# achao2013/deep3dmap

Measured on AMD Instinct MI355X. Metric: rendered Mpix/s fwd+bwd, 100k-tri mesh @512x512, higher is better.
Workload: dtype f32

## Files before the change

deep3dmap_amd/csrc/d3m_face_major.h:

```cpp
#pragma once
#include "d3m_backward.h"
#include "d3m_forward.h"

namespace d3m {

#ifndef D3M_FM_MAX_BBOX_AREA
#define D3M_FM_MAX_BBOX_AREA 4096
#endif
constexpr int FM_MAX_BBOX_AREA = D3M_FM_MAX_BBOX_AREA;
constexpr int FM_LANES = 8;
constexpr int FM_FACES_PER_BLOCK = 256 / FM_LANES;

template <int N>
struct BoxCursorN {
    int x, y, x0, x1, bw;
    __device__ __forceinline__ BoxCursorN(int x0_, int x1_, int y0_, int start) : x0(x0_), x1(x1_), bw(x1_ - x0_ + 1) {
        y = y0_ + start / bw;
        x = x0_ + start % bw;
    }
    __device__ __forceinline__ void advance() {
        x += N;
        while (x > x1) { x -= bw; y++; }
    }
};
typedef BoxCursorN<FM_LANES> BoxCursor;

__device__ __forceinline__ float quad_sum(float v) {
    static_assert(FM_LANES == 8, "quad_sum is written for 8 lanes per face");
    v += dpp_f32<0xB1>(v);
    v += dpp_f32<0x4E>(v);
    v += dpp_f32<0x141>(v);
    return v;
}
constexpr int FLAG_HIDDEN = 0, FLAG_VISIBLE = 1, FLAG_LARGE = 2;

__global__ void __launch_bounds__(256) k_mark_visible(const int32_t* __restrict__ face_index_map, int* __restrict__ flags,
                                                     int B, int F, int S) {
    const long i = (long)blockIdx.x * 256 + threadIdx.x;
    if (i >= (long)B * S * S) return;
    const int fi = face_index_map[i];
    if (fi >= 0) flags[(size_t)(i / ((long)S * S)) * F + fi] = FLAG_VISIBLE;
}

template <class FS, int LANES>
__device__ __forceinline__ void backward_depth_face(FS fs, const float* __restrict__ depth_map,
                                                    const int32_t* __restrict__ face_index_map,
                                                    const float* __restrict__ weight_map,
                                                    const float* __restrict__ grad_depth_map, float* __restrict__ grad_faces,
                                                    int* __restrict__ flags, int S, long gi, int sub, int F,
                                                    const VertexTarget& vt, int* __restrict__ n_large, int flip_rows,
                                                    int max_area) {
    const int bn = (int)(gi / F), fn = (int)(gi % F);
    float face[9], finv[9];
    fs.load(bn, fn, face);
    int x0, x1, y0, y1;
    if (!pixel_bbox(face, S, x0, x1, y0, y1)) return;
    const int area = (x1 - x0 + 1) * (y1 - y0 + 1);
    if (area > max_area) {
        flags[gi] = FLAG_LARGE;
        if (n_large && sub == 0) atomicAdd(n_large, 1);
        return;
    }
    face_inverse(face, S, finv);
    float tmp[3] = {0, 0, 0};
#pragma unroll
    for (int k = 0; k < 3; k++) {
#pragma unroll
        for (int l = 0; l < 3; l++) tmp[k] += -finv[3 * l + k] / face[3 * l + 2];
    }
    float acc[9] = {0, 0, 0, 0, 0, 0, 0, 0, 0};
    const size_t base = (size_t)bn * S * S;
    BoxCursorN<LANES> c(x0, x1, y0, sub);
    for (int i = sub; i < area; i += LANES, c.advance()) {
        const size_t p = base + (size_t)c.y * S + c.x;
        const bool own = face_index_map[p] == fn;
        const float ld = depth_map[p], lg = grad_depth_map[flip_rows ? base + (size_t)(S - 1 - c.y) * S + c.x : p];
        const float lw[3] = {weight_map[3 * p], weight_map[3 * p + 1], weight_map[3 * p + 2]};
        if (!__builtin_amdgcn_ballot_w64(own)) continue;
        const float depth = own ? ld : 1.0f, g = own ? lg : 0.0f;
        const float depth2 = depth * depth;
#pragma unroll
        for (int k = 0; k < 3; k++) {
            const float wk = own ? lw[k] : 0.0f, z_k = face[3 * k + 2];
            acc[3 * k + 0] += -g * tmp[0] * wk * depth2 * (float)S / 2.0f;
            acc[3 * k + 1] += -g * tmp[1] * wk * depth2 * (float)S / 2.0f;
            acc[3 * k + 2] += g * wk * depth2 / (z_k * z_k);
        }
    }
#pragma unroll
    for (int k = 0; k < 9; k++) acc[k] = LANES == 64 ? wave_sum(acc[k]) : quad_sum(acc[k]);
    if (sub == 0) {
        if (vt.gv) {
#pragma unroll
            for (int v = 0; v < 3; v++) {
                float* g = vt.vertex(bn, fn, v);
#pragma unroll
                for (int k = 0; k < 3; k++) atomicAdd(&g[k], acc[3 * v + k]);
            }
        } else {
            float* gf = grad_faces + (size_t)gi * 9;
#pragma unroll
            for (int k = 0; k < 9; k++) gf[k] += acc[k];
        }
    }
}

template <class FS, int LANES = FM_LANES>
__global__ void __launch_bounds__(256) k_backward_depth_faces(FS fs, const float* __restrict__ depth_map,
                                                             const int32_t* __restrict__ face_index_map,
                                                             const float* __restrict__ weight_map,
                                                             const float* __restrict__ grad_depth_map,
                                                             float* __restrict__ grad_faces, int* __restrict__ flags, int B,
                                                             int S, const int* __restrict__ list,
                                                             const int* __restrict__ n_list, VertexTarget vt,
                                                             int* __restrict__ n_large, int flip_rows, int max_area) {
    static_assert(LANES == FM_LANES || LANES == 64, "eight lanes per face, or a wave");
    const int sub = threadIdx.x % LANES;
    const int F = fs.num_faces();
    const long n_units = list ? (long)*n_list : (long)B * F;
    for (long u = (long)blockIdx.x * (256 / LANES) + threadIdx.x / LANES; u < n_units; u += (long)gridDim.x * (256 / LANES)) {
        const long gi = list ? (long)list[u] : u;
        if (!list && flags[gi] == FLAG_HIDDEN) continue;
        backward_depth_face<FS, LANES>(fs, depth_map, face_index_map, weight_map, grad_depth_map, grad_faces, flags, S, gi, sub, F, vt,
                            n_large, flip_rows, max_area);
    }
}

template <class FS>
__global__ void __launch_bounds__(256) k_backward_textures_faces(FS fs, const int32_t* __restrict__ face_index_map,
                                                                const float* __restrict__ sampling_weight_map,
                                                                const int32_t* __restrict__ sampling_index_map,
                                                                const float* __restrict__ grad_rgb_map,
                                                                float* __restrict__ grad_textures, int* __restrict__ flags,
                                                                int B, int S) {
    __shared__ float s_acc[24][256];
    const long gi = (long)blockIdx.x * FM_FACES_PER_BLOCK + threadIdx.x / FM_LANES;
    const int sub = threadIdx.x % FM_LANES;
    const int F = fs.num_faces();
    if (gi >= (long)B * F || flags[gi] == FLAG_HIDDEN) return;
    const int bn = (int)(gi / F), fn = (int)(gi % F);
    float face[9];
    fs.load(bn, fn, face);
    int x0, x1, y0, y1;
    if (!pixel_bbox(face, S, x0, x1, y0, y1)) return;
    const int area = (x1 - x0 + 1) * (y1 - y0 + 1);
    if (area > FM_MAX_BBOX_AREA) { flags[gi] = FLAG_LARGE; return; }
    const int l = threadIdx.x;
#pragma unroll
    for (int t = 0; t < 24; t++) s_acc[t][l] = 0;
    const size_t base = (size_t)bn * S * S;
    BoxCursor c(x0, x1, y0, sub);
    for (int i = sub; i < area; i += FM_LANES, c.advance()) {
        const size_t p = base + (size_t)c.y * S + c.x;
        if (face_index_map[p] != fn) continue;
        const float g0 = grad_rgb_map[3 * p + 0], g1 = grad_rgb_map[3 * p + 1], g2 = grad_rgb_map[3 * p + 2];
#pragma unroll
        for (int pn = 0; pn < 8; pn++) {
            const float w = sampling_weight_map[p * 8 + pn];
            const int isc = sampling_index_map[p * 8 + pn] & 7;
            s_acc[isc * 3 + 0][l] += w * g0;
            s_acc[isc * 3 + 1][l] += w * g1;
            s_acc[isc * 3 + 2][l] += w * g2;
        }
    }
    __builtin_amdgcn_fence(__ATOMIC_RELEASE, "wavefront");
    __builtin_amdgcn_wave_barrier();
    __builtin_amdgcn_fence(__ATOMIC_ACQUIRE, "wavefront");
    if (sub == 0) {
        float* gt = grad_textures + (size_t)gi * 24;
#pragma unroll
        for (int t = 0; t < 24; t++) {
            float v = s_acc[t][l];
#pragma unroll
            for (int j = 1; j < FM_LANES; j++) v += s_acc[t][l + j];
            gt[t] += v;
        }
    }
}

}
```

deep3dmap_amd/csrc/d3m_lit.h:

```cpp
#pragma once
#include "d3m_aux.h"
#include "d3m_tail.h"
#include "d3m_face_major.h"

namespace d3m {

struct LitTextures {
    const float* textures;
    const float* light;
    int F, Fp, ts, tex_batch, light_batch, fill_back;
    const float* im;
    int im_H, im_W;
};

__device__ __forceinline__ long lit_texel(const LitTextures& t, int B, int b, int fp, int isc, int* light_row) {
    const int ts3 = t.ts * t.ts * t.ts;
    long vf = (long)b * t.Fp + fp + isc / ts3;
    isc %= ts3;
    if (vf >= (long)B * t.Fp) return -1;
    const int bb = (int)(vf / t.Fp), ff = (int)(vf % t.Fp);
    *light_row = (t.light_batch > 1 ? bb : 0) * t.Fp + ff;
    int fo = ff, idx = isc;
    if (ff >= t.F) {
        fo = ff - t.F;
// ... 616 lines not shown
        }
    }
    const float4 t = block_sum4_256(make_float4(t_rgb, t_d, t_m, t_sse), s_part);
    if (threadIdx.x == 0)
        reinterpret_cast<float4*>(fit.partials)[((size_t)blockIdx.z * gridDim.y + blockIdx.y) * gridDim.x + blockIdx.x] = t;
}

template <int TILE>
__global__ void __launch_bounds__(256) k_fit_loss_records(const float* __restrict__ rgb_im, const float* __restrict__ depth_im,
                                                         const float* __restrict__ alpha_im,
                                                         const int32_t* __restrict__ face_index_map, int B, int S,
                                                         FitTargets fit, FitRecords rec) {
    constexpr int ROWS = 256 / TILE;
    __shared__ float4 s_part[4];
    __shared__ int s_col_lo_inv[TILE], s_col_hi1[TILE];
    if (threadIdx.x < TILE) { s_col_lo_inv[threadIdx.x] = 0; s_col_hi1[threadIdx.x] = 0; }
    __syncthreads();
    const int b = blockIdx.z, x0 = blockIdx.x * TILE, y0 = blockIdx.y * TILE;
    const int tx = threadIdx.x % TILE, ty = threadIdx.x / TILE;
    const float inv_pixels = 1.0f / (float)((long)S * S), inv_3den = 1.0f / (3.0f * *rec.mask_sum);
    float t_rgb = 0, t_d = 0, t_m = 0, t_sse = 0;
    auto sgn = [](float x) { return x > 0 ? 1.0f : (x < 0 ? -1.0f : 0.0f); };
    for (int r = ty; r < TILE; r += ROWS) {
        const int yi = y0 + r, xi = x0 + tx;
        bool nz = false;
        if (yi < S && xi < S) {
            const int yo = S - 1 - yi;
            const size_t p = ((size_t)b * S + yi) * S + xi, o = ((size_t)b * S + yo) * S + xi;
            float tg[6], v[3];
#pragma unroll
            for (int k = 0; k < 3; k++) {
                tg[k] = fit.rgb_t[(((size_t)b * 3 + k) * S + yo) * S + xi];
                v[k] = rgb_im[(((size_t)b * 3 + k) * S + yo) * S + xi];
            }
            tg[3] = fit.depth_t[o]; tg[4] = fit.alpha_t[o]; tg[5] = fit.mask[o];
            const int fi = face_index_map[p];
            const float depth = depth_im[o], alpha = alpha_im[o];
            const float m = tg[5], d = alpha - tg[4];
#pragma unroll
            for (int k = 0; k < 3; k++) t_rgb += fabsf(v[k] - tg[k]) * m;
            t_d += fabsf(depth - tg[3]) * m;
            t_m += m;
            t_sse += d * d;
            float4 g;
            g.x = (2.0f * d) * inv_pixels;
            g.y = (sgn(v[0] - tg[0]) * m) * inv_3den;
            g.z = (sgn(v[1] - tg[1]) * m) * inv_3den;
            g.w = (sgn(v[2] - tg[2]) * m) * inv_3den;
            float dot = alpha * g.x;
            dot += v[0] * g.y;
            dot += v[1] * g.z;
            dot += v[2] * g.w;
            rec.grad[p] = g;
            rec.dot[p] = make_float2(dot, __int_as_float(fi));
            rec.g_depth[p] = sgn(depth - tg[3]) * m;
            nz = g.x != 0 || g.y != 0 || g.z != 0 || g.w != 0 || dot != 0;
        }
        const unsigned half = tile_row_mask<TILE>(__ballot(nz));
        if (half != 0 && tx == 0) {
            const size_t line = ((size_t)b * 2 + 1) * S + (y0 + r);
            atomicMax(&rec.nz_lo_inv[line], S - (x0 + (__ffs((int)half) - 1)));
            atomicMax(&rec.nz_hi1[line], x0 + (32 - __clz((int)half)));
        }
        if (nz) {
            atomicMax(&s_col_lo_inv[tx], S - (y0 + r));
            atomicMax(&s_col_hi1[tx], y0 + r + 1);
        }
    }
    __syncthreads();
    if (threadIdx.x < TILE && s_col_hi1[threadIdx.x] != 0 && x0 + (int)threadIdx.x < S) {
        const size_t line = ((size_t)b * 2 + 0) * S + (x0 + threadIdx.x);
        atomicMax(&rec.nz_lo_inv[line], s_col_lo_inv[threadIdx.x]);
        atomicMax(&rec.nz_hi1[line], s_col_hi1[threadIdx.x]);
    }
    const float4 t = block_sum4_256(make_float4(t_rgb, t_d, t_m, t_sse), s_part);
    if (threadIdx.x == 0)
        reinterpret_cast<float4*>(fit.partials)[((size_t)blockIdx.z * gridDim.y + blockIdx.y) * gridDim.x + blockIdx.x] = t;
}

#ifndef D3M_LIT_LANES
#define D3M_LIT_LANES 8
#endif
constexpr int LIT_LANES = D3M_LIT_LANES;
constexpr int LIT_FACES_PER_BLOCK = 256 / LIT_LANES;
__device__ __forceinline__ float lit_sum(float v) {
    v += dpp_f32<0xB1>(v);
    v += dpp_f32<0x4E>(v);
    if (LIT_LANES == 8) v += dpp_f32<0x141>(v);
    return v;
}

struct LitFaceArgs {
    const float* faces;
    LitTextures lt;
    const int32_t* face_index_map;
    const float *weight_map, *depth_map;
    RgbGrad grad_rgb;
    float* gtex_view;
    float* grad_light;
    const float* grad_depth_map;
    float* grad_faces;
    VertexTarget vt;
    int* flags;
    unsigned* view_mask;
    const int* list;
    const int* n_list;
    int B, S;
    float eps;
    GradScale gs;
    int* n_large;
    int max_area = FM_MAX_BBOX_AREA;
};

template <int LANES>
__device__ __forceinline__ float lit_lanes_sum(float v) { return LANES == 64 ? wave_sum(v) : lit_sum(v); }
template <int LANES>
__device__ __forceinline__ void lit_face_backward(const LitFaceArgs& a, long gi, int sub) {
    const float* __restrict__ faces = a.faces;
    const LitTextures& lt = a.lt;
    const int32_t* __restrict__ face_index_map = a.face_index_map;
    const float* __restrict__ weight_map = a.weight_map;
    const float* __restrict__ depth_map = a.depth_map;
    const RgbGrad grad_rgb = a.grad_rgb;
    float* __restrict__ gtex_view = a.gtex_view;
    float* __restrict__ grad_light = a.grad_light;
    const float* __restrict__ grad_depth_map = a.grad_depth_map;
    float* __restrict__ grad_faces = a.grad_faces;
    const VertexTarget& vt = a.vt;
    int* __restrict__ flags = a.flags;
    const int S = a.S;
    const float eps = a.eps;
    const int Fp = lt.Fp;
    float s_rgb, s_alpha, s_depth;
    a.gs.get(s_rgb, s_alpha, s_depth);
    if (!a.list && flags[gi] == FLAG_HIDDEN) return;
    const int bn = (int)(gi / Fp), fn = (int)(gi % Fp);
    const float* face = faces + (size_t)gi * 9;
    float fc[9];
#pragma unroll
    for (int k = 0; k < 9; k++) fc[k] = face[k];
    int x0, x1, y0, y1;
    if (!pixel_bbox(fc, S, x0, x1, y0, y1)) return;
    const int area = (x1 - x0 + 1) * (y1 - y0 + 1);
    const int fo = fn >= lt.F ? fn - lt.F : fn;
    float* gt = gtex_view + ((size_t)bn * lt.F + fo) * 24;
    if (sub == 0 && a.view_mask) atomicOr(&a.view_mask[(size_t)fo * ((a.B + 31) >> 5) + (bn >> 5)], 1u << (bn & 31));
    if (area > a.max_area) {
        flags[gi] = FLAG_LARGE;
        if (sub == 0) atomicAdd(a.n_large, 1);
        for (int t = sub; t < 24; t += LANES) gt[t] = 0.0f;
        return;
    }
    float acc[24];
#pragma unroll
    for (int t = 0; t < 24; t++) acc[t] = 0.0f;
    const size_t base = (size_t)bn * S * S;
    float dacc[9] = {0, 0, 0, 0, 0, 0, 0, 0, 0}, dtmp[3] = {0, 0, 0};
    const float rz[3] = {__builtin_amdgcn_rcpf(fc[2]), __builtin_amdgcn_rcpf(fc[5]), __builtin_amdgcn_rcpf(fc[8])};
    if (grad_depth_map) {
        float px[3], py[3];
#pragma unroll
        for (int n = 0; n < 3; n++) { px[n] = to_pixel(fc[3 * n], S); py[n] = to_pixel(fc[3 * n + 1], S); }
        const float rden = __builtin_amdgcn_rcpf(px[2] * (py[0] - py[1]) + px[0] * (py[1] - py[2]) + px[1] * (py[2] - py[0]));
        const float ix[3] = {(py[1] - py[2]) * rden, (py[2] - py[0]) * rden, (py[0] - py[1]) * rden};
        const float iy[3] = {(px[2] - px[1]) * rden, (px[0] - px[2]) * rden, (px[1] - px[0]) * rden};
#pragma unroll
        for (int l2 = 0; l2 < 3; l2++) {
            dtmp[0] += -ix[l2] * rz[l2];
            dtmp[1] += -iy[l2] * rz[l2];
        }
    }
    const int lrow = (lt.light_batch > 1 ? bn : 0) * Fp + fn;
    const float li[3] = {lt.light[3 * (size_t)lrow], lt.light[3 * (size_t)lrow + 1], lt.light[3 * (size_t)lrow + 2]};
    constexpr int TPL = LANES >= 8 ? 1 : 8 / LANES;
    const float* tex_face = lt.textures + ((size_t)(lt.tex_batch > 1 ? bn : 0) * lt.F + fo) * 24;
    int to[TPL];
    float tx[TPL][3];
#pragma unroll
    for (int j = 0; j < TPL; j++) {
        const int t = (sub + j * LANES) & 7;
        to[j] = fn >= lt.F ? ((t & 1) << 2) | (t & 2) | ((t >> 2) & 1) : t;
#pragma unroll
        for (int c3 = 0; c3 < 3; c3++) tx[j][c3] = tex_face[to[j] * 3 + c3];
    }
    BoxCursorN<LANES> c(x0, x1, y0, sub);
    for (int i = sub; i < area; i += LANES, c.advance()) {
        const size_t p = base + (size_t)c.y * S + c.x;
        const bool own = face_index_map[p] == fn;
        const float lw0 = weight_map[3 * p], lw1 = weight_map[3 * p + 1], lw2 = weight_map[3 * p + 2];
        const float lg0 = grad_rgb.get(p, 0) * s_rgb, lg1 = grad_rgb.get(p, 1) * s_rgb, lg2 = grad_rgb.get(p, 2) * s_rgb;
        const float ld = depth_map[p], lgd = grad_depth_map ? grad_depth_map[p] * s_depth : 0.0f;
        if (!__builtin_amdgcn_ballot_w64(own)) continue;
        const float third = 1.0f / 3.0f;
        const float weight[3] = {own ? lw0 : third, own ? lw1 : third, own ? lw2 : third};
        const float g0 = own ? lg0 : 0.0f, g1 = own ? lg1 : 0.0f, g2 = own ? lg2 : 0.0f;
        const float depth = own ? ld : 1.0f;
        if (grad_depth_map) {
            const float g = own ? lgd : 0.0f, depth2 = depth * depth;
#pragma unroll
            for (int k = 0; k < 3; k++) {
                const float z_k = fc[3 * k + 2];
                dacc[3 * k + 0] += -g * dtmp[0] * weight[k] * depth2 * (float)S / 2.0f;
                dacc[3 * k + 1] += -g * dtmp[1] * weight[k] * depth2 * (float)S / 2.0f;
                dacc[3 * k + 2] += g * weight[k] * depth2 * (rz[k] * rz[k]);
            }
        }
        int fl[3] = {0, 0, 0};
        float fr[3];
#pragma unroll
        for (int k = 0; k < 3; k++) fr[k] = fminf(fmaxf(weight[k] * (depth * rz[k]), 0.0f), 1.0f - eps);
#pragma unroll
        for (int pn = 0; pn < 8; pn++) {
            float w;
            int isc_dyn;
            sample_corner(pn, 2, fl, fr, w, isc_dyn);
            const int isc = ((pn & 1) << 2) | (pn & 2) | ((pn >> 2) & 1);
            acc[isc * 3 + 0] += w * g0;
            acc[isc * 3 + 1] += w * g1;
            acc[isc * 3 + 2] += w * g2;
        }
    }
#pragma unroll
    for (int t = 0; t < 24; t++) acc[t] = lit_lanes_sum<LANES>(acc[t]);
    if (grad_depth_map) {
#pragma unroll
        for (int k = 0; k < 9; k++) dacc[k] = lit_lanes_sum<LANES>(dacc[k]);
        if (sub == 0) {
            if (vt.gv) {
#pragma unroll
                for (int n = 0; n < 3; n++) {
                    float* g = vt.vertex(bn, fn, n);
#pragma unroll
                    for (int k = 0; k < 3; k++) atomicAdd(&g[k], dacc[3 * n + k]);
                }
            } else {
                float* gf = grad_faces + (size_t)gi * 9;
#pragma unroll
                for (int k = 0; k < 9; k++) gf[k] += dacc[k];
            }
        }
    }
    float gl[3] = {0, 0, 0};
#pragma unroll
    for (int j = 0; j < TPL; j++) {
        float mine[3] = {0, 0, 0};
#pragma unroll
        for (int t = 0; t < 8; t++) {
            if (sub + j * LANES == t) { mine[0] = acc[3 * t]; mine[1] = acc[3 * t + 1]; mine[2] = acc[3 * t + 2]; }
        }
        if (sub + j * LANES < 8) {
#pragma unroll
            for (int c3 = 0; c3 < 3; c3++) {
                gt[to[j] * 3 + c3] = mine[c3] * li[c3];
                gl[c3] += mine[c3] * tx[j][c3];
            }
        }
    }
#pragma unroll
    for (int c3 = 0; c3 < 3; c3++) gl[c3] = lit_lanes_sum<LANES>(gl[c3]);
    if (grad_light && sub == 0) {
        atomicAdd(&grad_light[3 * (size_t)lrow + 0], gl[0]);
        atomicAdd(&grad_light[3 * (size_t)lrow + 1], gl[1]);
        atomicAdd(&grad_light[3 * (size_t)lrow + 2], gl[2]);
    }
}

template <int LANES = LIT_LANES>
__global__ void __launch_bounds__(256) k_backward_textures_lit_faces(LitFaceArgs a) {
    static_assert(LANES == LIT_LANES || LANES == 64, "LIT_LANES lanes per face, or a wave");
    constexpr int PER_BLOCK = 256 / LANES;
    const int sub = threadIdx.x % LANES, slot = threadIdx.x / LANES;
    if (a.list) {
        const int n = *a.n_list;
        const XcdOrder xo((n + PER_BLOCK - 1) / PER_BLOCK);
        for (int i = blockIdx.x; xo.more(i); i += gridDim.x) {
            const long base = (long)xo.unit(i) * PER_BLOCK;
            if (base + slot < n) lit_face_backward<LANES>(a, a.list[base + slot], sub);
        }
    } else {
        const long gi = (long)blockIdx.x * PER_BLOCK + slot;
        if (gi < (long)a.B * a.lt.Fp) lit_face_backward<LANES>(a, gi, sub);
    }
}

constexpr int LIT_ANY_MAX_TEXELS = 64;
template <int LANES>
__device__ __forceinline__ void lit_face_backward_any(const LitFaceArgs& a, long gi, int sub, float* __restrict__ acc_lds) {
    const LitTextures& lt = a.lt;
    const int S = a.S, Fp = lt.Fp, ts = lt.ts, ts3 = ts * ts * ts;
    float s_rgb, s_alpha, s_depth;
    a.gs.get(s_rgb, s_alpha, s_depth);
    const int bn = (int)(gi / Fp), fn = (int)(gi % Fp);
    float fc[9];
#pragma unroll
    for (int k = 0; k < 9; k++) fc[k] = a.faces[(size_t)gi * 9 + k];
    int x0, x1, y0, y1;
    if (!pixel_bbox(fc, S, x0, x1, y0, y1)) return;
    const int area = (x1 - x0 + 1) * (y1 - y0 + 1);
    const bool back = fn >= lt.F;
    const int fo = back ? fn - lt.F : fn;
    float* gt = a.gtex_view + ((size_t)bn * lt.F + fo) * ts3 * 3;
    if (sub == 0 && a.view_mask) atomicOr(&a.view_mask[(size_t)fo * ((a.B + 31) >> 5) + (bn >> 5)], 1u << (bn & 31));
    if (area > a.max_area) {
        a.flags[gi] = FLAG_LARGE;
        if (sub == 0) atomicAdd(a.n_large, 1);
        for (int t = sub; t < ts3 * 3; t += LANES) gt[t] = 0.0f;
        return;
    }
    for (int t = sub; t < ts3 * 3; t += LANES) acc_lds[t] = 0.0f;
    float dacc[9] = {0, 0, 0, 0, 0, 0, 0, 0, 0}, dtmp[3] = {0, 0, 0};
    if (a.grad_depth_map) {
        float finv[9];
        face_inverse(fc, S, finv);
#pragma unroll
        for (int k = 0; k < 3; k++) {
#pragma unroll
            for (int l = 0; l < 3; l++) dtmp[k] += -finv[3 * l + k] / fc[3 * l + 2];
        }
    }
    const int lrow = (lt.light_batch > 1 ? bn : 0) * Fp + fn;
    const float li[3] = {lt.light[3 * (size_t)lrow], lt.light[3 * (size_t)lrow + 1], lt.light[3 * (size_t)lrow + 2]};
    const float* tex_face = lt.textures + ((size_t)(lt.tex_batch > 1 ? bn : 0) * lt.F + fo) * ts3 * 3;
    __builtin_amdgcn_fence(__ATOMIC_RELEASE, "wavefront");
    __builtin_amdgcn_wave_barrier();
    const size_t base = (size_t)bn * S * S;
    BoxCursorN<LANES> c(x0, x1, y0, sub);
    for (int i = sub; i < area; i += LANES, c.advance()) {
        const size_t p = base + (size_t)c.y * S + c.x;
        const bool own = a.face_index_map[p] == fn;
        const float lw[3] = {a.weight_map[3 * p], a.weight_map[3 * p + 1], a.weight_map[3 * p + 2]};
        const float lg[3] = {a.grad_rgb.get(p, 0) * s_rgb, a.grad_rgb.get(p, 1) * s_rgb, a.grad_rgb.get(p, 2) * s_rgb};
        const float ld = a.depth_map[p], lgd = a.grad_depth_map ? a.grad_depth_map[p] * s_depth : 0.0f;
        if (!own) continue;
        if (a.grad_depth_map) {
            const float depth2 = ld * ld;
#pragma unroll
            for (int k = 0; k < 3; k++) {
                const float z_k = fc[3 * k + 2];
                dacc[3 * k + 0] += -lgd * dtmp[0] * lw[k] * depth2 * (float)S / 2.0f;
                dacc[3 * k + 1] += -lgd * dtmp[1] * lw[k] * depth2 * (float)S / 2.0f;
                dacc[3 * k + 2] += lgd * lw[k] * depth2 / (z_k * z_k);
            }
        }
        int fl[3];
        float fr[3];
        sample_setup(fc, lw, ld, ts, a.eps, fl, fr);
#pragma unroll
        for (int pn = 0; pn < 8; pn++) {
            float w;
            int isc;
            sample_corner(pn, ts, fl, fr, w, isc);
#pragma unroll
            for (int k = 0; k < 3; k++) atomicAdd(&acc_lds[isc * 3 + k], w * lg[k]);
        }
    }
    if (a.grad_depth_map) {
#pragma unroll
        for (int k = 0; k < 9; k++) dacc[k] = lit_lanes_sum<LANES>(dacc[k]);
        if (sub == 0) {
            if (a.vt.gv) {
#pragma unroll
                for (int n = 0; n < 3; n++) {
                    float* g = a.vt.vertex(bn, fn, n);
#pragma unroll
                    for (int k = 0; k < 3; k++) atomicAdd(&g[k], dacc[3 * n + k]);
                }
            } else {
                float* gf = a.grad_faces + (size_t)gi * 9;
#pragma unroll
                for (int k = 0; k < 9; k++) gf[k] += dacc[k];
            }
        }
    }
    __builtin_amdgcn_fence(__ATOMIC_RELEASE, "wavefront");
    __builtin_amdgcn_wave_barrier();
    __builtin_amdgcn_fence(__ATOMIC_ACQUIRE, "wavefront");
    float gl[3] = {0, 0, 0};
    for (int t = sub; t < ts3; t += LANES) {
        const int to = back ? (t % ts) * ts * ts + ((t / ts) % ts) * ts + t / (ts * ts) : t;
#pragma unroll
        for (int c3 = 0; c3 < 3; c3++) {
            const float m = acc_lds[t * 3 + c3];
            gt[to * 3 + c3] = m * li[c3];
            gl[c3] += m * tex_face[to * 3 + c3];
        }
    }
#pragma unroll
    for (int c3 = 0; c3 < 3; c3++) gl[c3] = lit_lanes_sum<LANES>(gl[c3]);
    if (a.grad_light && sub == 0) {
#pragma unroll
        for (int c3 = 0; c3 < 3; c3++) atomicAdd(&a.grad_light[3 * (size_t)lrow + c3], gl[c3]);
    }
}
template <int LANES = LIT_LANES>
__global__ void __launch_bounds__(256) k_backward_textures_lit_faces_any(LitFaceArgs a) {
    constexpr int PER_BLOCK = 256 / LANES;
    __shared__ float s_acc[PER_BLOCK][LIT_ANY_MAX_TEXELS * 3];
    const int sub = threadIdx.x % LANES, slot = threadIdx.x / LANES;
    const int n = *a.n_list;
    const XcdOrder xo((n + PER_BLOCK - 1) / PER_BLOCK);
    for (int i = blockIdx.x; xo.more(i); i += gridDim.x) {
        const long base = (long)xo.unit(i) * PER_BLOCK;
        if (base + slot < n) lit_face_backward_any<LANES>(a, a.list[base + slot], sub, s_acc[slot]);
    }
}

__device__ __forceinline__ void lit_large_flush(const LitTextures& lt, int B, float* __restrict__ gtex_view,
                                                float* __restrict__ grad_light, int bn, int fi, int lrow, const float* sums) {
#pragma unroll
    for (int pn = 0; pn < 8; pn++) {
        const int isc = ((pn & 1) << 2) | (pn & 2) | ((pn >> 2) & 1);
        int lr = 0;
        const long off = lit_texel(lt, B, bn, fi, isc, &lr);
        float* gt = gtex_view + (size_t)bn * lt.F * 24 + off % ((long)lt.F * 24);
#pragma unroll
        for (int k = 0; k < 3; k++) atomicAdd(&gt[k], sums[3 * pn + k]);
    }
    if (grad_light) {
#pragma unroll
        for (int k = 0; k < 3; k++) atomicAdd(&grad_light[3 * (size_t)lrow + k], sums[24 + k]);
    }
}

__device__ __forceinline__ void backward_textures_lit_pixels(const float* __restrict__ faces, const LitTextures& lt,
                                                             const int32_t* __restrict__ face_index_map,
                                                             const float* __restrict__ weight_map,
                                                             const float* __restrict__ depth_map, RgbGrad grad_rgb,
                                                             float* __restrict__ gtex_view ,
                                                             float* __restrict__ grad_light,
                                                             const int* __restrict__ only_large, int B, int S, float eps,
                                                             GradScale gs) {
    const long n = (long)B * S * S;
    __shared__ WgSums<27> wg;
    wg.init();
    const long chunk = ((n + gridDim.x - 1) / gridDim.x + 255) / 256 * 256;
    const long run_end = min(n, (long)(blockIdx.x + 1) * chunk);
    for (long i0 = (long)blockIdx.x * chunk + (threadIdx.x & ~63); i0 < run_end; i0 += 256) {
    const long i = i0 + (threadIdx.x & 63);
// ... 179 lines not shown
```

deep3dmap_amd/csrc/d3m_raster.hip:

```cpp
#include <hip/hip_runtime.h>
#include <stdint.h>
#include <stdio.h>
#include <string.h>

#include "../../include/d3m_raster.h"
#include "d3m_launch.h"
#include "d3m_aux.h"
#include "d3m_textures.h"
#include "d3m_vertex_colors.h"
#include "d3m_mesh_reg.h"
#include "d3m_morphable.h"
#include "d3m_pose.h"
#include "d3m_mesh.h"
#include "d3m_uv.h"
#include "d3m_backward.h"
#include "d3m_device.h"
#include "d3m_edge_grad.h"
#include "d3m_face_major.h"
#include "d3m_forward.h"
#include "d3m_lit.h"
#include "d3m_g2s.h"
#include "d3m_bid.h"
#include "d3m_front.h"
#include "d3m_light_grad.h"
// ... 1447 lines not shown
}
static int lit_clear_ranges(const LitWorkspace& W, float* grad_textures, int textures_batch, float* grad_light, int light_batch,
                            int B, int num_tri, int fill_back, int texture_size, bool has_visibility, void** ptr, size_t* bytes) {
    const size_t ts3 = (size_t)texture_size * texture_size * texture_size, view_elems = (size_t)num_tri * ts3 * 3;
    const int Fp = (fill_back ? 2 : 1) * num_tri;
    const bool gathered = texture_size == 2 || (has_visibility && texture_size >= 3 && texture_size <= 4);
    const bool skip_zero = gathered && textures_batch == 1;
    int n = 0;
    if (!skip_zero) { ptr[n] = textures_batch > 1 ? grad_textures : W.gview; bytes[n++] = (size_t)B * view_elems * 4; }
    if (grad_light) { ptr[n] = grad_light; bytes[n++] = (size_t)light_batch * Fp * 12; }
    if (gathered) {
        if (skip_zero) { ptr[n] = W.view_mask; bytes[n++] = W.mask_bytes + 256; }
        else { ptr[n] = W.n_large; bytes[n++] = 256; }
        if (!has_visibility) { ptr[n] = W.flags; bytes[n++] = (size_t)B * Fp * 4; }
    }
    return n;
}
D3M_EXPORT int d3m_backward_textures_lit_clear_ranges(float* grad_textures, int textures_batch, float* grad_light,
                                                      int light_batch, int batch_size, int num_tri, int fill_back,
                                                      int texture_size, void* workspace, int has_visibility, void** ptrs,
                                                      size_t* bytes) {
    if (batch_size <= 0 || num_tri <= 0 || texture_size <= 0 || !workspace || !ptrs || !bytes) return 0;
    const LitWorkspace W = lit_workspace(workspace, batch_size, num_tri, fill_back, texture_size);
    return lit_clear_ranges(W, grad_textures, textures_batch, grad_light, light_batch, batch_size, num_tri, fill_back,
                            texture_size, has_visibility != 0, ptrs, bytes);
}

D3M_EXPORT int d3m_backward_textures_lit(const float* faces, const float* textures, int textures_batch, const float* light,
                                         int light_batch, const int32_t* face_index_map, const float* weight_map,
                                         const float* depth_map, const float* grad_rgb_map, float* grad_textures,
                                         float* grad_light, const float* grad_depth_map, float* grad_faces, int batch_size,
                                         int num_tri, int fill_back, int image_size, int texture_size, float eps,
                                         void* workspace, size_t workspace_bytes, const d3m_vertex_target* vertex_target,
                                         void* visibility, const d3m_fit_targets* unscaled, int flags_in, d3m_stream_t stream) {
    if ((grad_depth_map != nullptr) != (grad_faces != nullptr || vertex_target != nullptr)) return D3M_ERR_INVALID;
    VertexTarget vt;
    if (int rcv = to_vertex_target(vertex_target, (fill_back ? 2 : 1) * num_tri, vt)) return rcv;
    const bool records = unscaled && unscaled->edge_grad;
    if (!faces || !face_index_map || !weight_map || !depth_map || (!grad_rgb_map && !records) || !grad_textures ||
        batch_size <= 0 || image_size <= 0)
        return D3M_ERR_INVALID;
    const RgbGrad grad_rgb = records ? RgbGrad{(const float*)unscaled->edge_grad, 4, 1} : RgbGrad{grad_rgb_map, 3, 0};
    LitTextures lt;
    int rc = make_lit(lt, textures, textures_batch, light, light_batch, num_tri, texture_size, fill_back, batch_size);
    if (rc) return rc;
    if (lt.im) return D3M_ERR_INVALID;
    if (!workspace || workspace_bytes < d3m_backward_textures_lit_workspace_bytes(batch_size, num_tri, fill_back, texture_size))
        return D3M_ERR_WORKSPACE;
    hipStream_t st = (hipStream_t)stream;
    const int B = batch_size, S = image_size;
    if (unscaled && !unscaled->scratch && !unscaled->edge_grad) return D3M_ERR_INVALID;
    const GradScale gs = to_grad_scale(unscaled, S);
    const size_t ts3 = (size_t)texture_size * texture_size * texture_size;
    const size_t view_elems = (size_t)num_tri * ts3 * 3;
    const LitWorkspace W = lit_workspace(workspace, B, num_tri, fill_back, texture_size);
    float* gview = textures_batch > 1 ? grad_textures : W.gview;
    int* flags = W.flags;
    const long n = (long)B * S * S, nf = (long)B * lt.Fp;
    unsigned* view_mask = W.view_mask;
    const bool gathered_any = visibility && texture_size >= 3 && texture_size <= 4;
    const bool skip_zero = (texture_size == 2 || gathered_any) && textures_batch == 1;
    if (!(flags_in & D3M_PRECLEARED)) {
        void* z_ptr[4];
        size_t z_bytes[4];
        const int nz = lit_clear_ranges(W, grad_textures, textures_batch, grad_light, light_batch, B, num_tri, fill_back,
                                        texture_size, visibility != nullptr, z_ptr, z_bytes);
        HIP_TRY(zero_ranges_async(z_ptr, z_bytes, nz, st));
    }
    const int* list = nullptr;
    const int* n_list = nullptr;
    if (visibility) {
        const VisibilityView v = visibility_view(visibility, nf);
        flags = v.flags; list = v.list; n_list = v.count;
    }
    if (texture_size == 2) {
        const bool use_mask = skip_zero;
        if (!visibility)
            LAUNCH("k_mark_visible", k_mark_visible, dim3(blocks_for(n, 256)), dim3(256), st, face_index_map, flags, B, lt.Fp, S);
        LitFaceArgs fa{faces, lt, face_index_map, weight_map, depth_map, grad_rgb, gview, grad_light, grad_depth_map,
                       grad_faces, vt, flags, use_mask ? view_mask : nullptr, list, n_list, B, S, eps, gs, W.n_large,
                       deterministic_mode() ? INT_MAX : FM_MAX_BBOX_AREA};
        const bool coarse = list && (double)S * S > 48.0 * (double)num_tri;
        const unsigned all_blocks = blocks_for(nf, coarse ? 4 : LIT_FACES_PER_BLOCK);
        const dim3 g_faces(list ? (all_blocks > 4096 ? 4096 : (all_blocks + 7) / 8 * 8) : all_blocks);
        if (coarse) LAUNCH("k_backward_textures_lit_faces", k_backward_textures_lit_faces<64>, g_faces, dim3(256), st, fa);
        else LAUNCH("k_backward_textures_lit_faces", k_backward_textures_lit_faces<>, g_faces, dim3(256), st, fa);
        FitFin fin;
        memset(&fin, 0, sizeof(fin));
        if (records && unscaled->scratch && unscaled->loss && (unscaled->flags & D3M_FIT_FINISH_DEFERRED))
            fin = fit_fin_of_tiles(unscaled, B, S);
        LAUNCH("k_lit_large_faces", k_lit_large_faces, dim3(px_grid(n, true)), dim3(256), st, faces, lt, face_index_map,
               weight_map, depth_map, grad_rgb, gview, grad_light, (const int*)flags, B, S, eps, gs, (const int*)W.n_large,
               grad_depth_map, grad_faces, vt, fin);
    } else if (gathered_any) {
        LitFaceArgs fa{faces, lt, face_index_map, weight_map, depth_map, grad_rgb, gview, grad_light, grad_depth_map,
                       grad_faces, vt, flags, skip_zero ? view_mask : nullptr, list, n_list, B, S, eps, gs, W.n_large,
                       deterministic_mode() ? INT_MAX : FM_MAX_BBOX_AREA};
        const bool coarse = (double)S * S > 48.0 * (double)num_tri;
        const unsigned all_blocks = blocks_for(nf, coarse ? 4 : LIT_FACES_PER_BLOCK);
        const dim3 g_faces(all_blocks > 4096 ? 4096 : (all_blocks + 7) / 8 * 8);
        if (coarse) LAUNCH("k_backward_textures_lit_faces", k_backward_textures_lit_faces_any<64>, g_faces, dim3(256), st, fa);
        else LAUNCH("k_backward_textures_lit_faces", k_backward_textures_lit_faces_any<>, g_faces, dim3(256), st, fa);
        FitFin fin;
        memset(&fin, 0, sizeof(fin));
        if (records && unscaled->scratch && unscaled->loss && (unscaled->flags & D3M_FIT_FINISH_DEFERRED))
            fin = fit_fin_of_tiles(unscaled, B, S);
        LAUNCH("k_lit_large_faces", k_lit_large_faces, dim3(px_grid(n, true)), dim3(256), st, faces, lt, face_index_map,
               weight_map, depth_map, grad_rgb, gview, grad_light, (const int*)flags, B, S, eps, gs, (const int*)W.n_large,
               grad_depth_map, grad_faces, vt, fin);
    } else {
        if (records && unscaled->scratch && unscaled->loss && (unscaled->flags & D3M_FIT_FINISH_DEFERRED)) {
            const FitFin fin = fit_fin_of_tiles(unscaled, B, S);
            LAUNCH("k_fit_finish", k_fit_finish, dim3(fin.n_groups), dim3(256), st, fin);
        }
        LAUNCH("k_backward_textures_lit_pixels", k_backward_textures_lit_pixels, dim3(px_grid(n, false)), dim3(256), st,
               faces, lt, face_index_map, weight_map, depth_map, grad_rgb, gview, grad_light, (const int*)nullptr, B, S, eps,
               gs, (const int*)nullptr);
        if (grad_depth_map) {
            DenseFaces fs{faces, lt.Fp};
            if (vt.gv) {
                LAUNCH("k_backward_depth_map", k_backward_depth_map<DenseFaces>, dim3(px_grid(n, false)), dim3(256), st, fs,
                       depth_map, face_index_map, (const float*)nullptr, weight_map, grad_depth_map, (float*)nullptr, B, S,
                       (const int*)nullptr, vt, gs);
            } else {
                if (unscaled) return D3M_ERR_INVALID;
                const int rc2 = run_backward_depth(fs, depth_map, face_index_map, (const float*)nullptr, weight_map,
                                                   grad_depth_map, grad_faces, B, S, flags, false, st);
                if (rc2) return rc2;
            }
        }
    }
    if (textures_batch == 1) {
        if ((texture_size == 2 || texture_size == 4) && skip_zero && (((uintptr_t)gview | (uintptr_t)grad_textures) & 15) == 0)
            LAUNCH("k_sum_over_views", k_sum_over_views_ts2, dim3(blocks_for((long)view_elems / 4, 256)), dim3(256), st,
                   (const float4*)gview, (float4*)grad_textures, (long)view_elems / 4, B, (const unsigned*)view_mask,
                   (int)(ts3 * 3 / 4));
        else
            LAUNCH("k_sum_over_views", k_sum_over_views, dim3(blocks_for((long)view_elems, 256)), dim3(256), st,
                   (const float*)gview, grad_textures, (long)view_elems, B,
                   skip_zero ? (const int*)flags : (const int*)nullptr, num_tri, lt.Fp, (int)(ts3 * 3));
    }
    return check_launch();
}

D3M_EXPORT int d3m_output_epilogue(const int32_t* face_index_map, const float* rgb_map, const float* depth_map,
                                   const float* background, int background_batch, float* rgb_blended,
                                   float* alpha_map, float* rgb_out, float* alpha_out, float* depth_out, int batch_size,
                                   int image_size, int anti_aliasing, d3m_stream_t stream) {
    if (!face_index_map || batch_size <= 0 || image_size <= 0) return D3M_ERR_INVALID;
    if (anti_aliasing && (image_size & 1)) return D3M_ERR_INVALID;
    if (rgb_map && !background) return D3M_ERR_INVALID;
    if (background && background_batch != 1 && background_batch != batch_size) return D3M_ERR_INVALID;
    const int s = anti_aliasing ? image_size / 2 : image_size;
    const long n = (long)batch_size * s * s;
    LAUNCH("k_output_epilogue", k_output_epilogue, dim3(blocks_for(n, 256)), dim3(256), (hipStream_t)stream, face_index_map,
                       rgb_map, depth_map, background, background_batch, rgb_blended, alpha_map, rgb_out, alpha_out,
                       depth_out, batch_size, image_size, anti_aliasing ? 1 : 0);
    return check_launch();
}

D3M_EXPORT int d3m_output_epilogue_backward(const float* grad_rgb_out, const float* grad_alpha_out,
                                            const float* grad_depth_out, float* grad_rgb_map, float* grad_alpha_map,
                                            float* grad_depth_map, int batch_size, int image_size, int anti_aliasing,
                                            d3m_stream_t stream) {
    if (batch_size <= 0 || image_size <= 0) return D3M_ERR_INVALID;
    if ((grad_rgb_map && !grad_rgb_out) || (grad_alpha_map && !grad_alpha_out) || (grad_depth_map && !grad_depth_out))
        return D3M_ERR_INVALID;
// ... 788 lines not shown
```

Measured before the change: 5670.

## Compact owned pixels per face via ballot masks before backward accumulation

New measurement: 5813 (median of 6 runs). +2.5%, better.

```diff
diff --git a/deep3dmap_amd/csrc/d3m_face_major.h b/deep3dmap_amd/csrc/d3m_face_major.h
--- a/deep3dmap_amd/csrc/d3m_face_major.h
+++ b/deep3dmap_amd/csrc/d3m_face_major.h
@@ -1,4 +1,5 @@
 #pragma once
+#include <type_traits>
 #include "d3m_backward.h"
 #include "d3m_forward.h"
 
@@ -11,19 +12,77 @@
 constexpr int FM_LANES = 8;
 constexpr int FM_FACES_PER_BLOCK = 256 / FM_LANES;
 
-template <int N>
-struct BoxCursorN {
-    int x, y, x0, x1, bw;
-    __device__ __forceinline__ BoxCursorN(int x0_, int x1_, int y0_, int start) : x0(x0_), x1(x1_), bw(x1_ - x0_ + 1) {
-        y = y0_ + start / bw;
-        x = x0_ + start % bw;
-    }
-    __device__ __forceinline__ void advance() {
-        x += N;
-        while (x > x1) { x -= bw; y++; }
-    }
-};
-typedef BoxCursorN<FM_LANES> BoxCursor;
+
+__device__ __forceinline__ int nth_set_bit(uint32_t m, int n) {
+    int pos = 0, c = __popc(m & 0xFFFFu);
+    if (n >= c) { n -= c; pos = 16; m >>= 16; }
+    c = __popc(m & 0xFFu);
+    if (n >= c) { n -= c; pos += 8; m >>= 8; }
+    c = __popc(m & 0xFu);
+    if (n >= c) { n -= c; pos += 4; m >>= 4; }
+    c = __popc(m & 0x3u);
+    if (n >= c) { n -= c; pos += 2; m >>= 2; }
+    if (n >= (int)(m & 1u)) pos += 1;
+    return pos;
+}
+__device__ __forceinline__ int nth_set_bit(uint64_t m, int n) {
+    const uint32_t lo = (uint32_t)m, hi = (uint32_t)(m >> 32);
+    const int c = __popc(lo);
+    return n >= c ? 32 + nth_set_bit(hi, n - c) : nth_set_bit(lo, n);
+}
+
+__device__ __forceinline__ void box_split(int t, int bw, float rbw, int& q, int& r) {
+    q = (int)((float)t * rbw);
+    r = t - q * bw;
+    if (r < 0) { q--; r += bw; }
+    if (r >= bw) { q++; r -= bw; }
+}
+
+template <int LANES, class Body>
+__device__ __forceinline__ void scan_owned_pixels(const int32_t* __restrict__ fim_view, int fn, int S, int x0, int x1, int y0,
+                                                  int area, int sub, Body&& body) {
+    static_assert(LANES == 64 || (LANES <= 16 && 32 % LANES == 0), "a chunk is one 32-bit mask per group, or the wave's ballot");
+    constexpr int K = LANES == 64 ? 1 : 32 / LANES, CHUNK = LANES * K;
+    const int bw = x1 - x0 + 1;
+    const float rbw = __builtin_amdgcn_rcpf((float)bw);
+    const int shift = (int)(threadIdx.x & 63u) - sub;
+    int cr = 0, cy = y0;
+    auto request_owners = [&](int cb, int cr_, int cy_, int32_t* owner) {
+#pragma unroll
+        for (int k = 0; k < K; k++) {
+            const int o = k * LANES + sub;
+            int q, r;
+            box_split(cr_ + o, bw, rbw, q, r);
+            owner[k] = cb + o < area ? fim_view[(size_t)(cy_ + q) * S + (x0 + r)] : -1;
+        }
+    };
+    int32_t owner[K];
+    request_owners(0, cr, cy, owner);
+    for (int cb = 0; cb < area; cb += CHUNK) {
+        typename std::conditional<LANES == 64, uint64_t, uint32_t>::type m;
+        if constexpr (LANES == 64) {
+            m = __builtin_amdgcn_ballot_w64(owner[0] == fn);
+        } else {
+            m = 0;
+#pragma unroll
+            for (int k = 0; k < K; k++) {
+                const uint64_t bal = __builtin_amdgcn_ballot_w64(owner[k] == fn);
+                m |= ((uint32_t)(bal >> shift) & ((1u << LANES) - 1u)) << (k * LANES);
+            }
+        }
+        int nq, nr;
+        box_split(cr + CHUNK, bw, rbw, nq, nr);
+        if (cb + CHUNK < area) request_owners(cb + CHUNK, nr, cy + nq, owner);
+        const int cnt = LANES == 64 ? __popcll(m) : __popc((uint32_t)m);
+        for (int n = sub; n < cnt; n += LANES) {
+            int q, r;
+            box_split(cr + nth_set_bit(m, n), bw, rbw, q, r);
+            body(x0 + r, cy + q);
+        }
+        cy += nq;
+        cr = nr;
+    }
+}
 
 __device__ __forceinline__ float quad_sum(float v) {
     static_assert(FM_LANES == 8, "quad_sum is written for 8 lanes per face");
@@ -70,23 +129,19 @@
     }
     float acc[9] = {0, 0, 0, 0, 0, 0, 0, 0, 0};
     const size_t base = (size_t)bn * S * S;
-    BoxCursorN<LANES> c(x0, x1, y0, sub);
-    for (int i = sub; i < area; i += LANES, c.advance()) {
-        const size_t p = base + (size_t)c.y * S + c.x;
-        const bool own = face_index_map[p] == fn;
-        const float ld = depth_map[p], lg = grad_depth_map[flip_rows ? base + (size_t)(S - 1 - c.y) * S + c.x : p];
+    scan_owned_pixels<LANES>(face_index_map + base, fn, S, x0, x1, y0, area, sub, [&](int x, int y) {
+        const size_t p = base + (size_t)y * S + x;
+        const float depth = depth_map[p], g = grad_depth_map[flip_rows ? base + (size_t)(S - 1 - y) * S + x : p];
         const float lw[3] = {weight_map[3 * p], weight_map[3 * p + 1], weight_map[3 * p + 2]};
-        if (!__builtin_amdgcn_ballot_w64(own)) continue;
-        const float depth = own ? ld : 1.0f, g = own ? lg : 0.0f;
         const float depth2 = depth * depth;
 #pragma unroll
         for (int k = 0; k < 3; k++) {
-            const float wk = own ? lw[k] : 0.0f, z_k = face[3 * k + 2];
+            const float wk = lw[k], z_k = face[3 * k + 2];
             acc[3 * k + 0] += -g * tmp[0] * wk * depth2 * (float)S / 2.0f;
             acc[3 * k + 1] += -g * tmp[1] * wk * depth2 * (float)S / 2.0f;
             acc[3 * k + 2] += g * wk * depth2 / (z_k * z_k);
         }
-    }
+    });
 #pragma unroll
     for (int k = 0; k < 9; k++) acc[k] = LANES == 64 ? wave_sum(acc[k]) : quad_sum(acc[k]);
     if (sub == 0) {
@@ -149,10 +204,8 @@
 #pragma unroll
     for (int t = 0; t < 24; t++) s_acc[t][l] = 0;
     const size_t base = (size_t)bn * S * S;
-    BoxCursor c(x0, x1, y0, sub);
-    for (int i = sub; i < area; i += FM_LANES, c.advance()) {
-        const size_t p = base + (size_t)c.y * S + c.x;
-        if (face_index_map[p] != fn) continue;
+    scan_owned_pixels<FM_LANES>(face_index_map + base, fn, S, x0, x1, y0, area, sub, [&](int x, int y) {
+        const size_t p = base + (size_t)y * S + x;
         const float g0 = grad_rgb_map[3 * p + 0], g1 = grad_rgb_map[3 * p + 1], g2 = grad_rgb_map[3 * p + 2];
 #pragma unroll
         for (int pn = 0; pn < 8; pn++) {
@@ -162,7 +215,7 @@
             s_acc[isc * 3 + 1][l] += w * g1;
             s_acc[isc * 3 + 2][l] += w * g2;
         }
-    }
+    });
     __builtin_amdgcn_fence(__ATOMIC_RELEASE, "wavefront");
     __builtin_amdgcn_wave_barrier();
     __builtin_amdgcn_fence(__ATOMIC_ACQUIRE, "wavefront");
diff --git a/deep3dmap_amd/csrc/d3m_lit.h b/deep3dmap_amd/csrc/d3m_lit.h
--- a/deep3dmap_amd/csrc/d3m_lit.h
+++ b/deep3dmap_amd/csrc/d3m_lit.h
@@ -722,6 +722,10 @@
 #define D3M_LIT_LANES 8
 #endif
 constexpr int LIT_LANES = D3M_LIT_LANES;
+#ifndef D3M_LIT_LIST_BLOCKS
+#define D3M_LIT_LIST_BLOCKS 4096
+#endif
+constexpr unsigned LIT_LIST_BLOCKS = D3M_LIT_LIST_BLOCKS;
 constexpr int LIT_FACES_PER_BLOCK = 256 / LIT_LANES;
 __device__ __forceinline__ float lit_sum(float v) {
     v += dpp_f32<0xB1>(v);
@@ -810,33 +814,13 @@
             dtmp[1] += -iy[l2] * rz[l2];
         }
     }
-    const int lrow = (lt.light_batch > 1 ? bn : 0) * Fp + fn;
-    const float li[3] = {lt.light[3 * (size_t)lrow], lt.light[3 * (size_t)lrow + 1], lt.light[3 * (size_t)lrow + 2]};
-    constexpr int TPL = LANES >= 8 ? 1 : 8 / LANES;
-    const float* tex_face = lt.textures + ((size_t)(lt.tex_batch > 1 ? bn : 0) * lt.F + fo) * 24;
-    int to[TPL];
-    float tx[TPL][3];
-#pragma unroll
-    for (int j = 0; j < TPL; j++) {
-        const int t = (sub + j * LANES) & 7;
-        to[j] = fn >= lt.F ? ((t & 1) << 2) | (t & 2) | ((t >> 2) & 1) : t;
-#pragma unroll
-        for (int c3 = 0; c3 < 3; c3++) tx[j][c3] = tex_face[to[j] * 3 + c3];
-    }
-    BoxCursorN<LANES> c(x0, x1, y0, sub);
-    for (int i = sub; i < area; i += LANES, c.advance()) {
-        const size_t p = base + (size_t)c.y * S + c.x;
-        const bool own = face_index_map[p] == fn;
-        const float lw0 = weight_map[3 * p], lw1 = weight_map[3 * p + 1], lw2 = weight_map[3 * p + 2];
-        const float lg0 = grad_rgb.get(p, 0) * s_rgb, lg1 = grad_rgb.get(p, 1) * s_rgb, lg2 = grad_rgb.get(p, 2) * s_rgb;
-        const float ld = depth_map[p], lgd = grad_depth_map ? grad_depth_map[p] * s_depth : 0.0f;
-        if (!__builtin_amdgcn_ballot_w64(own)) continue;
-        const float third = 1.0f / 3.0f;
-        const float weight[3] = {own ? lw0 : third, own ? lw1 : third, own ? lw2 : third};
-        const float g0 = own ? lg0 : 0.0f, g1 = own ? lg1 : 0.0f, g2 = own ? lg2 : 0.0f;
-        const float depth = own ? ld : 1.0f;
+    scan_owned_pixels<LANES>(face_index_map + base, fn, S, x0, x1, y0, area, sub, [&](int x, int y) {
+        const size_t p = base + (size_t)y * S + x;
+        const float weight[3] = {weight_map[3 * p], weight_map[3 * p + 1], weight_map[3 * p + 2]};
+        const float g0 = grad_rgb.get(p, 0) * s_rgb, g1 = grad_rgb.get(p, 1) * s_rgb, g2 = grad_rgb.get(p, 2) * s_rgb;
+        const float depth = depth_map[p];
         if (grad_depth_map) {
-            const float g = own ? lgd : 0.0f, depth2 = depth * depth;
+            const float g = grad_depth_map[p] * s_depth, depth2 = depth * depth;
 #pragma unroll
             for (int k = 0; k < 3; k++) {
                 const float z_k = fc[3 * k + 2];
@@ -859,6 +843,19 @@
             acc[isc * 3 + 1] += w * g1;
             acc[isc * 3 + 2] += w * g2;
         }
+    });
+    const int lrow = (lt.light_batch > 1 ? bn : 0) * Fp + fn;
+    const float li[3] = {lt.light[3 * (size_t)lrow], lt.light[3 * (size_t)lrow + 1], lt.light[3 * (size_t)lrow + 2]};
+    constexpr int TPL = LANES >= 8 ? 1 : 8 / LANES;
+    const float* tex_face = lt.textures + ((size_t)(lt.tex_batch > 1 ? bn : 0) * lt.F + fo) * 24;
+    int to[TPL];
+    float tx[TPL][3];
+#pragma unroll
+    for (int j = 0; j < TPL; j++) {
+        const int t = (sub + j * LANES) & 7;
+        to[j] = fn >= lt.F ? ((t & 1) << 2) | (t & 2) | ((t >> 2) & 1) : t;
+#pragma unroll
+        for (int c3 = 0; c3 < 3; c3++) tx[j][c3] = tex_face[to[j] * 3 + c3];
     }
 #pragma unroll
     for (int t = 0; t < 24; t++) acc[t] = lit_lanes_sum<LANES>(acc[t]);
@@ -964,14 +961,11 @@
     __builtin_amdgcn_fence(__ATOMIC_RELEASE, "wavefront");
     __builtin_amdgcn_wave_barrier();
     const size_t base = (size_t)bn * S * S;
-    BoxCursorN<LANES> c(x0, x1, y0, sub);
-    for (int i = sub; i < area; i += LANES, c.advance()) {
-        const size_t p = base + (size_t)c.y * S + c.x;
-        const bool own = a.face_index_map[p] == fn;
+    scan_owned_pixels<LANES>(a.face_index_map + base, fn, S, x0, x1, y0, area, sub, [&](int x, int y) {
+        const size_t p = base + (size_t)y * S + x;
         const float lw[3] = {a.weight_map[3 * p], a.weight_map[3 * p + 1], a.weight_map[3 * p + 2]};
         const float lg[3] = {a.grad_rgb.get(p, 0) * s_rgb, a.grad_rgb.get(p, 1) * s_rgb, a.grad_rgb.get(p, 2) * s_rgb};
         const float ld = a.depth_map[p], lgd = a.grad_depth_map ? a.grad_depth_map[p] * s_depth : 0.0f;
-        if (!own) continue;
         if (a.grad_depth_map) {
             const float depth2 = ld * ld;
 #pragma unroll
@@ -993,7 +987,7 @@
 #pragma unroll
             for (int k = 0; k < 3; k++) atomicAdd(&acc_lds[isc * 3 + k], w * lg[k]);
         }
-    }
+    });
     if (a.grad_depth_map) {
 #pragma unroll
         for (int k = 0; k < 9; k++) dacc[k] = lit_lanes_sum<LANES>(dacc[k]);
diff --git a/deep3dmap_amd/csrc/d3m_raster.hip b/deep3dmap_amd/csrc/d3m_raster.hip
--- a/deep3dmap_amd/csrc/d3m_raster.hip
+++ b/deep3dmap_amd/csrc/d3m_raster.hip
@@ -1553,7 +1553,7 @@
                        deterministic_mode() ? INT_MAX : FM_MAX_BBOX_AREA};
         const bool coarse = list && (double)S * S > 48.0 * (double)num_tri;
         const unsigned all_blocks = blocks_for(nf, coarse ? 4 : LIT_FACES_PER_BLOCK);
-        const dim3 g_faces(list ? (all_blocks > 4096 ? 4096 : (all_blocks + 7) / 8 * 8) : all_blocks);
+        const dim3 g_faces(list ? (all_blocks > LIT_LIST_BLOCKS ? LIT_LIST_BLOCKS : (all_blocks + 7) / 8 * 8) : all_blocks);
         if (coarse) LAUNCH("k_backward_textures_lit_faces", k_backward_textures_lit_faces<64>, g_faces, dim3(256), st, fa);
         else LAUNCH("k_backward_textures_lit_faces", k_backward_textures_lit_faces<>, g_faces, dim3(256), st, fa);
         FitFin fin;
```
